# LPD-EPFL-ML/X-MAP

Measured on AMD Instinct MI355X. Metric: item_sim_pairs_per_s, higher is better.
Workload: dtype f64

## Files before the change

### include/xmap_hip.h

```cpp
#ifndef XMAP_HIP_H
#define XMAP_HIP_H
#include <stdint.h>

#ifdef __cplusplus
extern "C" {
#endif

#define XMAP_OK 0
#define XMAP_ERR_HIP -1
#define XMAP_ERR_ARG -2
#define XMAP_ERR_OVERFLOW -3
#define XMAP_ERR_CAPACITY -4

#define XMAP_COSINE 0
#define XMAP_ADJUST_COSINE 1
#define XMAP_COSINE_EXACT 2

#define XMAP_TOPC 10

typedef struct xmap_ratings {
    int64_t n_users;
    int32_t n_items;
    int64_t nnz;
    const int64_t *user_ptr;
// ... 156 lines not shown
    const int32_t *mutu;
    const int32_t *nij;
    const double *info;
    const double *frac;
} xmap_sim;

int xmap_bridge_flags(void *stream, const xmap_sim *S, const int32_t *prefix_cls, uint8_t *bb);

int xmap_knn_classify(void *stream, const xmap_sim *S, int top_k, const uint8_t *bb, const int32_t *suffix_cls,
                      const uint32_t *contains_mask, uint8_t *cls, int32_t *kcnt ,
                      int32_t *kcol , double *kval ,
                      int32_t row_lo, int32_t row_hi );

int xmap_knn_thresholds(void *stream, int32_t n_items, int top_k, const int32_t *kcnt, const int32_t *kcol, const double *kval,
                        void *thr );
int xmap_reverse_count(void *stream, const xmap_sim *S, int mode, int top_k, const uint8_t *bb, const uint8_t *cls,
                       const int32_t *kcnt, const int32_t *kcol, const double *kval, const int32_t *suffix_cls,
                       const uint32_t *contains_mask, const uint8_t *flags, const int64_t *attach_ptr,
                       const void *thr ,
                       int32_t *long_rows ,
                       uint8_t *eflag ,
                       int32_t *rcnt , int32_t row_lo, int32_t row_hi );
int xmap_reverse_count_att_rnn(void *stream, const xmap_sim *S, int top_k, const uint8_t *bb, const uint8_t *cls,
                               const int32_t *kcnt, const int32_t *kcol, const double *kval, const int32_t *suffix_cls,
                               const uint32_t *contains_mask, const uint8_t *flags, const void *thr, int32_t *long_rows,
                               uint8_t *eflag, int32_t *rcnt_att , int32_t *rcnt_rnn , int32_t row_lo, int32_t row_hi);
int xmap_reverse_fill(void *stream, const xmap_sim *S, int mode, int top_k, const uint8_t *bb, const uint8_t *cls,
                      const int32_t *kcnt, const int32_t *kcol, const double *kval, const int32_t *suffix_cls,
                      const uint32_t *contains_mask, const uint8_t *flags, const int64_t *attach_ptr,
                      const void *thr ,
                      int32_t *long_rows ,
                      uint8_t *eflag , const int64_t *rptr ,
                      int32_t *ridx, double *rval , uint8_t *rflag, int32_t row_lo, int32_t row_hi);

typedef struct xmap_ext_tables {
    int32_t n_items, top_k;
    const uint8_t *cls; const int32_t *kcnt; const int32_t *kcol; const double *kval; const uint8_t *flags;
    const int64_t *att_ptr; const int32_t *att_idx; const double *att_val;
    const int64_t *src_ptr; const int32_t *src_idx; const double *src_val; const uint8_t *src_flag;
    const int64_t *rnn_ptr; const int32_t *rnn_idx; const double *rnn_val;
    int32_t n_nb; const int32_t *nb_id; const int32_t *nb_list; const void *midX; const void *dir; const int64_t *dir_ptr;
    int32_t n_ends; const int32_t *urank; const int32_t *uitem;
} xmap_ext_tables;
typedef struct xmap_path_units {
    int32_t n_units; const int32_t *unit_start; const int32_t *unit_c; const int32_t *unit_G; const int32_t *unit_row;
    int32_t *unit_nt; int32_t n_heavy; const int32_t *heavy_unit0;
// ... 500 lines not shown
```

### x-map_amd/csrc/api.hip

```cpp
#include <math.h>
#include <stdlib.h>
#include <algorithm>
#include <vector>

#include "common.h"
#include "rec_model.h"

namespace xmap {

struct Pool {
    std::vector<void *> ptrs;
    void release() {
        for (void *p : ptrs) (void)hipFree(p);
        ptrs.clear();
    }
};
struct ScratchPool : Pool { ~ScratchPool() { release(); } };

}

using namespace xmap;

struct xmap_ctx {
    int device = 0;
// ... 135 lines not shown

static void drop_labels(xmap_ctx *c) {
    c->p_lab.release();
    c->have_lab = false;
    c->n_labels = 0; c->n_lab = 0;
    c->h_lab_ptr.clear();
}

static void drop_fold(xmap_ctx *c) {
    c->p_fold.release();
    c->have_fold = false;
    c->f_users = c->f_rows = 0;
}

static int reverse_list(xmap_ctx *c, int mode, const uint8_t *bb, const int64_t *attach_ptr, const void *thr, int32_t *long_rows,
                        uint8_t *eflag, int32_t *counted ,
                        const int64_t **rptr, const int32_t **ridx, const double **rval, const uint8_t **rflag) {
    const int I = c->R.n_items, k = c->top_k;
    int32_t *rcnt = counted;
    int64_t *ptr;
    XM_ALLOCZ(c->p_ext, ptr, I + 1);
    if (!counted) {
        XM_ALLOCZ(c->p_ext, rcnt, I);
        XM_TRY(xmap_reverse_count(c->st, &c->S, mode, k, bb, c->T.cls, c->T.kcnt, c->T.kcol, c->T.kval, c->R.suffix_cls,
                                  c->R.contains_mask, c->R.flags, attach_ptr, thr, long_rows, eflag, rcnt, 0, I));
    }
    int64_t n = 0;
    XM_TRY(xmap_exclusive_scan_i32_to_i64(c->st, rcnt, ptr, I, &n));
    int32_t *idx;
    double *val;
    uint8_t *flag;
    XM_ALLOC(c->p_ext, idx, n);
    XM_ALLOC(c->p_ext, val, 3 * (size_t)(n ? n : 1));
    XM_ALLOCZ(c->p_ext, flag, n);
    XM_TRY(xmap_reverse_fill(c->st, &c->S, mode, k, bb, c->T.cls, c->T.kcnt, c->T.kcol, c->T.kval, c->R.suffix_cls,
                             c->R.contains_mask, c->R.flags, attach_ptr, thr, long_rows, eflag, ptr, idx, val, flag, 0, I));
    *rptr = ptr; *ridx = idx; *rval = val; *rflag = flag;
    return XMAP_OK;
}

static int ensure_rows(xmap_ctx *c, int64_t slots, int64_t len, int64_t hrows) {
    if (c->acc == nullptr || c->acc_slots < slots || c->acc_len != len || c->hacc_rows < hrows) {
        c->p_rows.release();
        c->acc = nullptr; c->hacc = nullptr;
        XM_ALLOCZ(c->p_rows, c->acc, (size_t)slots * len * 4);
        XM_ALLOC(c->p_rows, c->touched, (size_t)slots * len);
        if (hrows) {
            XM_ALLOCZ(c->p_rows, c->hacc, (size_t)hrows * len * 4);
            XM_ALLOC(c->p_rows, c->htouched, (size_t)hrows * len);
        }
        c->acc_slots = slots; c->acc_len = len; c->hacc_rows = hrows;
// ... 340 lines not shown
    XM_ALLOCZ(c->p_ext, c->top_val, (size_t)I * XMAP_TOPC);
    c->n_out = c->n_paths = 0;
    if (I == 0) { c->have_ext = true; if (n_out) *n_out = 0; if (n_paths) *n_paths = 0; return XMAP_OK; }
    uint8_t *bb, *cls;
    int32_t *kcnt, *kcol;
    double *kval;
    XM_ALLOCZ(c->p_ext, bb, I); XM_ALLOC(c->p_ext, cls, I); XM_ALLOC(c->p_ext, kcnt, (size_t)I * 2);
    XM_ALLOC(c->p_ext, kcol, (size_t)I * 2 * k); XM_ALLOC(c->p_ext, kval, (size_t)I * 2 * k * 3);
    XM_TRY(xmap_bridge_flags(c->st, &c->S, c->R.prefix_cls, bb));
    XM_TRY(xmap_knn_classify(c->st, &c->S, k, bb, c->R.suffix_cls, c->R.contains_mask, cls, kcnt, kcol, kval, 0, I));
    T.cls = cls; T.kcnt = kcnt; T.kcol = kcol; T.kval = kval;
    XM_TRY(xmap_edge_ranges(c->st, &c->S, &c->fast_div));
    double *thr;
    int32_t *long_rows;
    XM_ALLOC(c->p_ext, thr, (size_t)I * 4);
    XM_ALLOC(c->p_ext, long_rows, I + 1);
    uint8_t *eflag;
    XM_ALLOC(c->p_ext, eflag, (size_t)(c->n_kept > 0 ? c->n_kept : 1));
    XM_TRY(xmap_knn_thresholds(c->st, I, k, kcnt, kcol, kval, thr));
    const uint8_t *dummy;
    int32_t *cnt_att, *cnt_rnn;
    XM_ALLOCZ(c->p_ext, cnt_att, I);
    XM_ALLOCZ(c->p_ext, cnt_rnn, I);
    XM_TRY(xmap_reverse_count_att_rnn(c->st, &c->S, k, bb, cls, kcnt, kcol, kval, c->R.suffix_cls, c->R.contains_mask, c->R.flags,
                                      thr, long_rows, eflag, cnt_att, cnt_rnn, 0, I));
    XM_TRY(reverse_list(c, 0, bb, nullptr, thr, long_rows, eflag, cnt_att, &T.att_ptr, &T.att_idx, &T.att_val, &dummy));
    XM_TRY(reverse_list(c, 2, bb, nullptr, thr, long_rows, eflag, cnt_rnn, &T.rnn_ptr, &T.rnn_idx, &T.rnn_val, &dummy));
    XM_TRY(reverse_list(c, 1, bb, T.att_ptr, thr, long_rows, eflag, nullptr, &T.src_ptr, &T.src_idx, &T.src_val, &T.src_flag));
    int64_t *wtmp, *P;
    XM_ALLOCZ(c->p_ext, wtmp, (size_t)4 * I); XM_ALLOCZ(c->p_ext, P, I);
    XM_TRY(xmap_path_weights(c->st, &T, wtmp, P));
    int32_t *nb_list, *nb_id;
    int64_t n_nb = 0;
    XM_ALLOC(c->p_ext, nb_list, I); XM_ALLOC(c->p_ext, nb_id, I);
    XM_TRY(xmap_nb_index(c->st, I, cls, nb_list, nb_id, &n_nb));
    T.n_nb = (int32_t)n_nb; T.nb_list = nb_list; T.nb_id = nb_id;
    if (n_nb > 0) {
        int32_t *ng;
        int64_t *nrec, *dir_ptr, *rec_ptr, n_tiles = 0, n_records = 0;
        void *dir, *midX;
        XM_ALLOC(c->p_ext, ng, n_nb); XM_ALLOC(c->p_ext, nrec, n_nb); XM_ALLOCZ(c->p_ext, dir_ptr, n_nb + 1); XM_ALLOCZ(c->p_ext, rec_ptr, n_nb + 1);
        XM_TRY(xmap_mid_rows_count(c->st, &T, ng, nrec));
        XM_TRY(xmap_exclusive_scan_i32_to_i64(c->st, ng, dir_ptr, n_nb, &n_tiles));
// ... 1655 lines not shown
```

### x-map_amd/csrc/reverse.hip

```cpp
#include "paths.h"
#include <stdlib.h>

namespace xmap {

struct RevArgs {
    int I, k, mode;
    int row_lo, row_hi;
    const KnnThr *thr;
    const int *long_rows;
    uint8_t *eflag;
    int rev_long;
    const long long *row_ptr;
    const int *col;
    const double *sim;
    const int *mutu;
    const int *nij;
    const double *info;
    const double *frac;
    const uint8_t *bb;
    const uint8_t *cls;
    const int *kcnt;
    const int *kcol;
    const double *kval;
    const int *suffix_cls;
// ... 73 lines not shown
        if (p < hi) A.eflag[p - p0] = (uint8_t)((ok ? (A.mode == 2 ? 4 : 1) : 0) | (fl << 1));
        return ok;
    }
    b = 0; sv = 0.0; fl = 0;
    bool ok = false;
    if (p < hi) {
        const uint8_t e = A.eflag[p - p0];
        ok = (e & (A.mode == 2 ? 4 : 1)) != 0;
        fl = (uint8_t)((e >> 1) & 1);
        if (ok) { b = A.col[p]; sv = A.sim[p]; }
    }
    return ok;
}

constexpr int REV_LONG = 4096;
constexpr int REV_WAVES = 16;
template <bool FILL>
__global__ __launch_bounds__(256) void k_reverse(RevArgs A) {
    int a = A.row_lo + blockIdx.x * 4 + (threadIdx.x >> 6);
    if (a >= A.row_hi) return;
    int lane = lane_id();
    long long lo = A.row_ptr[a], hi = A.row_ptr[a + 1];
    if (A.long_rows && hi - lo > A.rev_long) return;
    bool row_ok = true;
    if (A.mode == 1) row_ok = (A.flags[a] & 2) != 0;
    long long out = FILL ? A.rptr[a] : 0;
    int total = 0, total2 = 0;
    const long long p0 = A.eflag ? A.row_ptr[A.row_lo] : 0;
    if (row_ok)
        for (long long base = lo; base < hi; base += 64) {
            long long p = base + lane;
            int b; double sv; uint8_t fl;
            const bool ok = rev_test<FILL>(A, a, p, hi, p0, b, sv, fl);
            unsigned long long m = __ballot(ok);
            if (FILL && ok) rev_write(A, a, p, out + __popcll(m & lanemask_lt()), b, sv, fl);
            int c = __popcll(m);
            out += c;
            total += c;
            if (!FILL && A.mode == 3) total2 += __popcll(__ballot((fl & 2) != 0));
        }
    if (!FILL && lane == 0) { A.rcnt[a] = total; if (A.mode == 3) A.rcnt2[a] = total2; }
}

__global__ __launch_bounds__(256) void k_rev_long_rows(int row_lo, int row_hi, const long long *row_ptr, int rev_long,
                                                       int *long_rows ) {
    const int a = row_lo + blockIdx.x * blockDim.x + threadIdx.x;
    if (a < row_hi && row_ptr[a + 1] - row_ptr[a] > rev_long) long_rows[1 + atomicAdd(&long_rows[0], 1)] = a;
}

template <bool FILL>
__global__ __launch_bounds__(64 * REV_WAVES) void k_reverse_long(RevArgs A) {
    __shared__ int s_cnt[REV_WAVES];
    __shared__ int s_tot2;
    const int lane = lane_id(), w = threadIdx.x >> 6;
    const int n_long = A.long_rows[0];
    const long long p0 = A.eflag ? A.row_ptr[A.row_lo] : 0;
    for (int r = blockIdx.x; r < n_long; r += gridDim.x) {
        const int a = A.long_rows[1 + r];
        const long long lo = A.row_ptr[a], hi = A.row_ptr[a + 1];
        const bool row_ok = (A.mode != 1) || ((A.flags[a] & 2) != 0);
        long long out = FILL ? A.rptr[a] : 0;
        int total = 0, total2 = 0;
        if (!FILL && A.mode == 3) { if (threadIdx.x == 0) s_tot2 = 0; __syncthreads(); }
        if (row_ok)
            for (long long base = lo; base < hi; base += 64 * REV_WAVES) {
                const long long p = base + threadIdx.x;
                int b; double sv; uint8_t fl;
                const bool ok = rev_test<FILL>(A, a, p, hi, p0, b, sv, fl);
                const unsigned long long m = __ballot(ok);
                if (!FILL && A.mode == 3) total2 += __popcll(__ballot((fl & 2) != 0));
                if (lane == 0) s_cnt[w] = __popcll(m);
                __syncthreads();
                int before = 0, all = 0;
                for (int o = 0; o < REV_WAVES; o++) { const int c = s_cnt[o]; if (o < w) before += c; all += c; }
                if (FILL && ok) rev_write(A, a, p, out + before + __popcll(m & lanemask_lt()), b, sv, fl);
                out += all;
                total += all;
                __syncthreads();
            }
        if (!FILL && A.mode == 3) {
            if (lane == 0) atomicAdd(&s_tot2, total2);
            __syncthreads();
            if (threadIdx.x == 0) A.rcnt2[a] = s_tot2;
            __syncthreads();
        }
        if (!FILL && threadIdx.x == 0) A.rcnt[a] = total;
    }
}

}

using namespace xmap;

extern "C" {

static int reverse_common(void *stream, bool fill, const xmap_sim *S, int mode, int top_k, const uint8_t *bb,
                          const uint8_t *cls, const int32_t *kcnt, const int32_t *kcol, const double *kval,
                          const int32_t *suffix_cls, const uint32_t *contains_mask, const uint8_t *flags,
                          const int64_t *attach_ptr, const void *thr, int32_t *long_rows, uint8_t *eflag, int32_t *rcnt,
                          const int64_t *rptr, int32_t *ridx, double *rval, uint8_t *rflag, int32_t row_lo, int32_t row_hi,
                          int32_t *rcnt2 = nullptr) {
    XM_ARG(S && bb && cls && kcnt && kcol && kval && suffix_cls && contains_mask && flags);
    XM_ARG((mode >= 0 && mode <= 2) || (mode == 3 && !fill && rcnt2 && eflag));
    XM_ARG(mode != 1 || attach_ptr);
    XM_ARG(row_lo >= 0 && row_lo <= row_hi && row_hi <= S->n_items);
    if (row_hi == row_lo) return XMAP_OK;
    RevArgs A;
    A.I = S->n_items; A.k = top_k; A.mode = mode; A.thr = (const KnnThr *)thr; A.long_rows = long_rows; A.eflag = eflag;
    A.row_lo = row_lo; A.row_hi = row_hi;
    const char *rl = getenv("XMAP_REV_LONG");
    A.rev_long = (rl && atoi(rl) > 0) ? atoi(rl) : REV_LONG;
    A.row_ptr = (const long long *)S->row_ptr; A.col = S->col; A.sim = S->sim; A.mutu = S->mutu; A.nij = S->nij;
    A.info = S->info; A.frac = S->frac; A.bb = bb; A.cls = cls; A.kcnt = kcnt; A.kcol = kcol; A.kval = kval;
    A.suffix_cls = suffix_cls; A.contains_mask = contains_mask; A.flags = flags;
    A.attach_ptr = (const long long *)attach_ptr;
    A.rcnt2 = rcnt2;
    A.rcnt = rcnt; A.rptr = (const long long *)rptr; A.ridx = ridx; A.rval = rval; A.rflag = rflag;
    const int n_rows = row_hi - row_lo;
    dim3 grid((unsigned)((n_rows + 3) / 4)), block(256);
    hipStream_t st = (hipStream_t)stream;

    if (long_rows && !fill) {
        XM_HIP(hipMemsetAsync(long_rows, 0, sizeof(int32_t), st));
        k_rev_long_rows<<<dim3((unsigned)((n_rows + 255) / 256)), dim3(256), 0, st>>>(row_lo, row_hi, (const long long *)S->row_ptr,
                                                                                  A.rev_long, long_rows);
        XM_LAUNCH_CHECK();
    }
    if (fill) k_reverse<true><<<grid, block, 0, st>>>(A);
    else k_reverse<false><<<grid, block, 0, st>>>(A);
    XM_LAUNCH_CHECK();
    if (long_rows) {
        if (fill) k_reverse_long<true><<<dim3(512), dim3(64 * REV_WAVES), 0, st>>>(A);
        else k_reverse_long<false><<<dim3(512), dim3(64 * REV_WAVES), 0, st>>>(A);
        XM_LAUNCH_CHECK();
    }
    return XMAP_OK;
}

int xmap_reverse_count(void *stream, const xmap_sim *S, int mode, int top_k, const uint8_t *bb, const uint8_t *cls,
                       const int32_t *kcnt, const int32_t *kcol, const double *kval, const int32_t *suffix_cls,
                       const uint32_t *contains_mask, const uint8_t *flags, const int64_t *attach_ptr, const void *thr,
                       int32_t *long_rows, uint8_t *eflag, int32_t *rcnt, int32_t row_lo, int32_t row_hi) {
    XM_ARG(rcnt);
    return reverse_common(stream, false, S, mode, top_k, bb, cls, kcnt, kcol, kval, suffix_cls, contains_mask, flags,
                          attach_ptr, thr, long_rows, eflag, rcnt, nullptr, nullptr, nullptr, nullptr, row_lo, row_hi);
}

int xmap_reverse_count_att_rnn(void *stream, const xmap_sim *S, int top_k, const uint8_t *bb, const uint8_t *cls,
                               const int32_t *kcnt, const int32_t *kcol, const double *kval, const int32_t *suffix_cls,
                               const uint32_t *contains_mask, const uint8_t *flags, const void *thr, int32_t *long_rows,
                               uint8_t *eflag, int32_t *rcnt_att, int32_t *rcnt_rnn, int32_t row_lo, int32_t row_hi) {
    XM_ARG(rcnt_att && rcnt_rnn && eflag);
    return reverse_common(stream, false, S, 3, top_k, bb, cls, kcnt, kcol, kval, suffix_cls, contains_mask, flags, nullptr, thr,
                          long_rows, eflag, rcnt_att, nullptr, nullptr, nullptr, nullptr, row_lo, row_hi, rcnt_rnn);
}

int xmap_reverse_fill(void *stream, const xmap_sim *S, int mode, int top_k, const uint8_t *bb, const uint8_t *cls,
                      const int32_t *kcnt, const int32_t *kcol, const double *kval, const int32_t *suffix_cls,
                      const uint32_t *contains_mask, const uint8_t *flags, const int64_t *attach_ptr, const void *thr,
                      int32_t *long_rows, uint8_t *eflag, const int64_t *rptr, int32_t *ridx, double *rval, uint8_t *rflag,
                      int32_t row_lo, int32_t row_hi) {
    XM_ARG(rptr && ridx && rval);
    return reverse_common(stream, true, S, mode, top_k, bb, cls, kcnt, kcol, kval, suffix_cls, contains_mask, flags,
                          attach_ptr, thr, long_rows, eflag, nullptr, rptr, ridx, rval, rflag, row_lo, row_hi);
}

}
```

### x-map_amd/csrc/util.hip

```cpp
#include <stdarg.h>
#include <stdlib.h>
#include <vector>

#include "common.h"

namespace xmap {
static thread_local char g_err[512] = "";
void set_error(const char *fmt, ...) {
    va_list ap;
    va_start(ap, fmt);
    vsnprintf(g_err, sizeof(g_err), fmt, ap);
    va_end(ap);
}

namespace {
struct Chunk { char *base; size_t size, used; };
struct Arena { int dev; hipStream_t st; std::vector<Chunk> chunks; size_t live; };
thread_local std::vector<Arena> g_arenas;
constexpr size_t ARENA_KEEP = (size_t)256 << 20;
Arena *arena_find(int dev, hipStream_t st) {
    for (Arena &a : g_arenas) if (a.dev == dev && a.st == st) return &a;
    return nullptr;
}
Arena *arena_of(hipStream_t st) {
// ... 252 lines not shown
            XM_LAUNCH_CHECK();
        }
        XM_HIP(xm_free_async(tile, st));
    }
    if (h_total) {
        XM_HIP(hipMemcpyAsync(h_total, out0 + n, sizeof(int64_t), hipMemcpyDeviceToHost, st));
        if (n_arrays == 2) XM_HIP(hipMemcpyAsync(h_total + 1, out1 + n, sizeof(int64_t), hipMemcpyDeviceToHost, st));
        XM_HIP(hipStreamSynchronize(st));
    }
    return XMAP_OK;
}
}

extern "C" {
const char *xmap_last_error(void) { return xmap::g_err; }
int xmap_version(void) { return 125; }

int xmap_trim(void) {
    XM_HIP(hipDeviceSynchronize());
    int dev = 0;
    XM_HIP(hipGetDevice(&dev));
    for (xmap::Arena &a : xmap::g_arenas) {
        if (a.dev != dev || a.live != 0) continue;
        for (xmap::Chunk &c : a.chunks) (void)hipFree(c.base);
        a.chunks.clear();
    }
    return XMAP_OK;
}

int xmap_debug_arena(void *stream, int64_t *live, int64_t *reserved) {
    XM_ARG(live && reserved);
// ... 38 lines not shown
```

### x-map_amd/xmap/engine/device.py

```python
import ctypes as C
import math
import os

import numpy as np
import torch

from . import hipabi as abi
from .exactness import plain_sums_exact

lib = abi.lib
vp, i32, i64, check = abi.vp, abi.i32, abi.i64, abi.check


def _stream(dev):
    return C.c_void_p(torch.cuda.current_stream(dev).cuda_stream)


SLOT_TARGET = 768
CH_MIN = 2048
STEPWISE = os.environ.get("XMAP_STAGE_A_STEPWISE") == "1"


class DeviceRatings(object):

# ... 748 lines not shown
        E.cls = alloc(max(I, 1), torch.uint8)
        E.kcnt = alloc((max(I, 1), 2), torch.int32)
        E.kcol = alloc((max(I, 1), 2, k), torch.int32)
        E.kval = alloc((max(I, 1), 2, k, 3), torch.float64)
        with self.timed("knn_classify"):
            lo, hi = (0, I) if rows is None else (int(rows[0]), int(rows[1]))
            check(lib.xmap_knn_classify(st, C.byref(S.c), k, vp(E.bb), vp(R.suffix_cls), vp(R.contains_mask),
                                        vp(E.cls), vp(E.kcnt), vp(E.kcol), vp(E.kval), i32(lo), i32(hi)))
        return E

    def _reverse(self, S, E, mode, attach_ptr):
        st8 = self.reverse_count(S, E, mode, attach_ptr, None)
        self.reverse_fill(st8)
        return st8.out

    def reverse_count(self, S, E, mode, attach_ptr, rows):
        R = self.R
        I = R.n_items
        st8 = ExtResult()
        st8.S, st8.E, st8.mode = S, E, mode
        st8.rows = (0, I) if rows is None else (int(rows[0]), int(rows[1]))
        st8.rcnt = self._zeros(max(I, 1), torch.int32)
        st8.eflag = self._empty(max(int(S.col.numel()), 1), torch.uint8)
        st8.args = (C.byref(S.c), mode, E.k, vp(E.bb), vp(E.cls), vp(E.kcnt), vp(E.kcol), vp(E.kval),
                    vp(R.suffix_cls), vp(R.contains_mask), vp(R.flags), vp(attach_ptr), vp(getattr(E, "thr", None)),
                    vp(getattr(E, "long_rows", None)), vp(st8.eflag))
        st8.keep = attach_ptr
        check(lib.xmap_reverse_count(_stream(self.dev), *st8.args, vp(st8.rcnt), i32(st8.rows[0]), i32(st8.rows[1])))
        return st8

    def reverse_count_pair(self, S, E, rows):
        R = self.R
        I = R.n_items
        lo, hi = (0, I) if rows is None else (int(rows[0]), int(rows[1]))
        eflag = self._empty(max(int(S.col.numel()), 1), torch.uint8)
        sts = []
        for mode in (0, 2):
            st8 = ExtResult()
            st8.S, st8.E, st8.mode, st8.rows = S, E, mode, (lo, hi)
            st8.rcnt = self._zeros(max(I, 1), torch.int32)
            st8.eflag = eflag
            st8.args = (C.byref(S.c), mode, E.k, vp(E.bb), vp(E.cls), vp(E.kcnt), vp(E.kcol), vp(E.kval),
                        vp(R.suffix_cls), vp(R.contains_mask), vp(R.flags), vp(None), vp(E.thr),
                        vp(getattr(E, "long_rows", None)), vp(eflag))
            st8.keep = None
            sts.append(st8)
        check(lib.xmap_reverse_count_att_rnn(_stream(self.dev), C.byref(S.c), E.k, vp(E.bb), vp(E.cls), vp(E.kcnt), vp(E.kcol),
                                             vp(E.kval), vp(R.suffix_cls), vp(R.contains_mask), vp(R.flags), vp(E.thr),
                                             vp(getattr(E, "long_rows", None)), vp(eflag), vp(sts[0].rcnt), vp(sts[1].rcnt),
                                             i32(lo), i32(hi)))
        return sts

    def reverse_gather_counts(self, sts, comm):
        I = self.R.n_items
        lo, hi = sts[0].rows
        for st8, c in zip(sts, comm.all_gather_multi([st8.rcnt[lo:hi] for st8 in sts])):
            st8.rcnt[:I] = c

    def reverse_fill(self, st8):
        I = self.R.n_items
        st = _stream(self.dev)
        rptr = self._zeros(I + 1, torch.int64)
        tot = C.c_int64(0)
        check(lib.xmap_exclusive_scan_i32_to_i64(st, vp(st8.rcnt), vp(rptr), i64(I), C.byref(tot)))
# ... 242 lines not shown
        lo, hi = rows
        with self.timed("knn_gather"):
            k = E.k
            fd = torch.tensor([E.fast_div], dtype=torch.int64, device=self.dev)
            comm.all_reduce(fd, "min")
            E.fast_div = int(fd.item())
            cls, kcnt, kcol, kval = comm.all_gather_multi([E.cls[lo:hi], E.kcnt[lo:hi].reshape(-1), E.kcol[lo:hi].reshape(-1),
                                                           E.kval[lo:hi].reshape(-1)])
            E.cls[:I] = cls
            E.kcnt[:I] = kcnt.view(I, 2)
            E.kcol[:I] = kcol.view(I, 2, k)
            E.kval[:I] = kval.view(I, 2, k, 3)
        E.rows = None
        return E

    def ext_thresholds(self, E):
        I = self.R.n_items
        E.thr = self._empty(max(I, 1) * 4, torch.float64)
        check(lib.xmap_knn_thresholds(_stream(self.dev), i32(I), E.k, vp(E.kcnt), vp(E.kcol), vp(E.kval), vp(E.thr)))
        E.long_rows = self._empty(max(I, 1) + 1, torch.int32)

    def ext_reverse(self, S, E):
        with self.timed("reverse"):
            self.ext_thresholds(E)
            if getattr(E, "thr", None) is not None and os.environ.get("XMAP_REV_SEPARATE") != "1":
                st_att, st_rnn = self.reverse_count_pair(S, E, None)
                self.reverse_fill(st_att)
                self.reverse_fill(st_rnn)
                E.att, E.rnn = st_att.out, st_rnn.out
            else:
                E.att = self._reverse(S, E, 0, None)
                E.rnn = self._reverse(S, E, 2, None)
            E.src = self._reverse(S, E, 1, E.att[0])
        return E

    def ext_tables_from_knn(self, top_k, cls, kcnt, kcol, kval):
        R = self.R
        I, k = R.n_items, int(top_k)
        dev = self.dev
# ... 1174 lines not shown
```

### x-map_amd/xmap/engine/hipabi.py

```python
import ctypes as C
import os

HERE = os.path.dirname(os.path.abspath(__file__))
LIB_PATH = os.environ.get("XMAP_HIP_LIB") or os.path.normpath(os.path.join(HERE, "..", "..", "libxmap_hip.so"))
XLIB_PATH = os.environ.get("XMAP_HIP_XLIB") or os.path.normpath(os.path.join(HERE, "..", "..", "libxmap_hip_xcheck.so"))

COSINE, ADJUST_COSINE = 0, 1
METHODS = {"cosine": COSINE, "adjust_cosine": ADJUST_COSINE}
COSINE_EXACT = 2
TOPC = 10
MID_ROWS_SPAN = 36864
ERR_HIP, ERR_ARG, ERR_OVERFLOW, ERR_CAPACITY = -1, -2, -3, -4
TOPN_KEEP_HELD = 1
AUDIENCE_KEEP_HOLDERS = 1
SRC_RESIDENT, SRC_FOLDIN, SRC_ITEM_FOLDIN = 0, 1, 2
GROUP_MEAN, GROUP_MIN, GROUP_MAX = 0, 1, 2
GROUP_MAX_MEMBERS = 64
PEERS_SAME, PEERS_KEEP_SELF, PEERS_CENTRED = 1, 2, 4
UKNN_OWN_MEAN, UKNN_KEEP_HELD = 1, 2
RELATED_SUM, RELATED_MEAN, RELATED_MAX = 0, 1, 2
RELATED_KEEP_MEMBERS = 1
RELATED_HOW = {"sum": RELATED_SUM, "mean": RELATED_MEAN, "max": RELATED_MAX}
POP_COUNT, POP_MEAN = 0, 1
FILL_WINDOW = 4096
# ... 74 lines not shown

class RecFilter(C.Structure):
    _fields_ = [("allow", C.c_void_p), ("ex_ptr", C.c_void_p), ("ex_id", C.c_void_p), ("min_score", C.c_double)]


class FuseList(C.Structure):
    _fields_ = [("cnt", C.c_void_p), ("item", C.c_void_p), ("score", C.c_void_p), ("width", C.c_int32), ("weight", C.c_double)]


EXPORTS = [
    "xmap_last_error", "xmap_version", "xmap_trim", "xmap_debug_arena", "xmap_debug_arena_call", "xmap_debug_sort_pairs", "xmap_debug_record_chunks", "xmap_exclusive_scan_i64", "xmap_exclusive_scan_i32_to_i64",
    "xmap_exclusive_scan2_i32_to_i64", "xmap_scan_self_tiles", "xmap_sim3_plan_begin", "xmap_sim3_plan_wait", "xmap_sim3_counters_begin", "xmap_sim3_counters_wait",
    "xmap_build_csc", "xmap_user_stats", "xmap_item_stats", 
    "xmap_sim2_layout", "xmap_sim2_plan", "xmap_sim2_units",
    "xmap_sim2_pairs", "xmap_sim2_scatter", "xmap_sim3_layout", "xmap_sim3_plan", "xmap_sim3_mircount", "xmap_sim3_mirror", "xmap_item_partials", "xmap_item_merge", "xmap_sim2_pack_partials",
    "xmap_sim2_sort_partials", "xmap_sim2_merge_partials", "xmap_sim2_pack_pairs", "xmap_sim2_unpack_pairs", "xmap_bridge_flags", "xmap_knn_classify", "xmap_knn_thresholds", "xmap_reverse_count", "xmap_reverse_count_att_rnn",
    "xmap_reverse_fill", "xmap_topc_from_lists", "xmap_path_weights", "xmap_extend_paths", 
    "xmap_mid_rows_count", "xmap_mid_rows_place", "xmap_edge_ranges", "xmap_end_universe", "xmap_extend_cols", "xmap_extend_cols_slots", "xmap_nb_index", "xmap_path_plan", "xmap_end_order", "xmap_dense_normalize", "xmap_dense_layout", "xmap_dense_topk", "xmap_rec_select", "xmap_predict", "xmap_rec_profiles", "xmap_predict_rows", "xmap_mae", "xmap_topn_rows", "xmap_audience_rows", "xmap_explain_rows", "xmap_explain_sources", "xmap_eval_users", "xmap_topn_eval", "xmap_select_map", "xmap_alterego_count", "xmap_alterego_fill", "xmap_foldin_count", "xmap_foldin_fill", "xmap_union_count", "xmap_union_fill",
    "xmap_feed_text", "xmap_feed_texts", "xmap_feed_merge", "xmap_feed_sizes", "xmap_feed_arrays", "xmap_feed_ids", "xmap_feed_free",
    "xmap_ctx_upload_feed", "xmap_feed_format", "xmap_ctx_create", "xmap_ctx_destroy", "xmap_check_ratings", "xmap_ctx_upload_ratings", "xmap_ctx_item_sim", "xmap_ctx_sim_download", "xmap_ctx_extend",
    "xmap_ctx_ext_download", "xmap_ctx_ext_lists", "xmap_ctx_candidates", "xmap_ctx_generate", "xmap_ctx_gen_download",
    "xmap_ctx_rec_sim", "xmap_ctx_rec_profiles_download", "xmap_ctx_rec_download", "xmap_ctx_rec_select", "xmap_ctx_rec_set_neighbors",
    "xmap_ctx_rec_neighbors_download", "xmap_ctx_predict", "xmap_ctx_recommend", "xmap_ctx_evaluate_topn",
    "xmap_ctx_foldin", "xmap_ctx_foldin_download", "xmap_ctx_foldin_recommend", "xmap_ctx_foldin_predict", "xmap_ctx_union",
    "xmap_ctx_explain", "xmap_ctx_foldin_explain", "xmap_ctx_audience", "xmap_ctx_foldin_audience",
    "xmap_itemfold_count", "xmap_itemfold_fill", "xmap_itemfold_audience_rows", "xmap_ctx_item_foldin", "xmap_ctx_item_foldin_download",
    "xmap_ctx_item_foldin_audience", "xmap_ctx_item_foldin_predict", "xmap_ctx_item_foldin_recommend",
    "xmap_topn_rows_filtered", "xmap_audience_rows_filtered", "xmap_ctx_recommend_filtered", "xmap_ctx_audience_filtered",
    "xmap_div_index", "xmap_diversify_rows", "xmap_ctx_recommend_diverse",
    "xmap_group_topn_rows", "xmap_ctx_recommend_group",
    "xmap_peer_index", "xmap_peer_centre", "xmap_peer_rows", "xmap_ctx_peers", "xmap_peer_rows_ls", "xmap_ctx_peers_ls",
# ... 135 lines not shown
```

### x-map_amd/xmap/engine/sharded.py

```python
import os

import numpy as np
import torch


def balanced_ranges(weights, world):
    w = np.asarray(weights, dtype=np.float64)
    n = len(w)
    c = np.concatenate([[0.0], np.cumsum(w)])
    total = c[-1]
    cuts = [0]
    for r in range(1, world):
        target = total * r / world
        cuts.append(int(min(max(np.searchsorted(c, target, side="left"), cuts[-1]), n)))
    cuts.append(n)
    return [(cuts[r], cuts[r + 1]) for r in range(world)]


def unit_cuts(c, w_heavy, world):
    n = int(c.numel())
    if n == 0:
        return np.zeros(world + 1, np.int64)
    wh = w_heavy if w_heavy is not None else torch.zeros((), dtype=torch.float64, device=c.device)
    first = torch.minimum(((c[-1] + wh) / world - wh).clamp(min=0.0), c[-1])
# ... 314 lines not shown
            err = e
        comm.agree(err, "stage B (mirror)")
        if share is not None:
            comm.all_reduce(bb, "max")
        err = None
        try:
            E = eng.ext_knn(S, k, comm, rows=share, bb=bb)
        except Exception as e:
            err = e
        comm.agree(err, "stage B (knn tables)")
        eng.ext_gather(E, comm)
        rows = getattr(E, "row_share", None)
        with eng.timed("reverse"):
            err = None
            try:
                eng.ext_thresholds(E)
            except Exception as e:
                err = e
            comm.agree(err, "stage B (list thresholds)")
            for group in (((0, "att"), (2, "rnn")), ((1, "src"),)):
                err, sts = None, []
                try:
                    if len(group) == 2:
                        sts = eng.reverse_count_pair(S, E, rows)
                    else:
                        for mode, _ in group:
                            sts.append(eng.reverse_count(S, E, mode, E.att[0] if mode == 1 else None, rows))
                except Exception as e:
                    err = e
                comm.agree(err, "stage B (reverse lists: count)")
                if rows is not None:
# ... 25 lines not shown
```

Baseline: 28.86 billion.

## Split long reverse-list rows into fixed segments processed by independent waves

```diff
diff --git a/include/xmap_hip.h b/include/xmap_hip.h
--- a/include/xmap_hip.h
+++ b/include/xmap_hip.h
@@ -194,22 +194,23 @@
 
 int xmap_knn_thresholds(void *stream, int32_t n_items, int top_k, const int32_t *kcnt, const int32_t *kcol, const double *kval,
                         void *thr );
+int xmap_reverse_scratch_len(int32_t n_items, int64_t n_entries, int64_t *h_len);
 int xmap_reverse_count(void *stream, const xmap_sim *S, int mode, int top_k, const uint8_t *bb, const uint8_t *cls,
                        const int32_t *kcnt, const int32_t *kcol, const double *kval, const int32_t *suffix_cls,
                        const uint32_t *contains_mask, const uint8_t *flags, const int64_t *attach_ptr,
                        const void *thr ,
-                       int32_t *long_rows ,
+                       int32_t *long_rows , int64_t long_len ,
                        uint8_t *eflag ,
                        int32_t *rcnt , int32_t row_lo, int32_t row_hi );
 int xmap_reverse_count_att_rnn(void *stream, const xmap_sim *S, int top_k, const uint8_t *bb, const uint8_t *cls,
                                const int32_t *kcnt, const int32_t *kcol, const double *kval, const int32_t *suffix_cls,
                                const uint32_t *contains_mask, const uint8_t *flags, const void *thr, int32_t *long_rows,
-                               uint8_t *eflag, int32_t *rcnt_att , int32_t *rcnt_rnn , int32_t row_lo, int32_t row_hi);
+                               int64_t long_len, uint8_t *eflag, int32_t *rcnt_att , int32_t *rcnt_rnn , int32_t row_lo, int32_t row_hi);
 int xmap_reverse_fill(void *stream, const xmap_sim *S, int mode, int top_k, const uint8_t *bb, const uint8_t *cls,
                       const int32_t *kcnt, const int32_t *kcol, const double *kval, const int32_t *suffix_cls,
                       const uint32_t *contains_mask, const uint8_t *flags, const int64_t *attach_ptr,
                       const void *thr ,
-                      int32_t *long_rows ,
+                      int32_t *long_rows , int64_t long_len,
                       uint8_t *eflag , const int64_t *rptr ,
                       int32_t *ridx, double *rval , uint8_t *rflag, int32_t row_lo, int32_t row_hi);
 
diff --git a/x-map_amd/csrc/api.hip b/x-map_amd/csrc/api.hip
--- a/x-map_amd/csrc/api.hip
+++ b/x-map_amd/csrc/api.hip
@@ -173,7 +173,7 @@
 }
 
 static int reverse_list(xmap_ctx *c, int mode, const uint8_t *bb, const int64_t *attach_ptr, const void *thr, int32_t *long_rows,
-                        uint8_t *eflag, int32_t *counted ,
+                        int64_t long_len, uint8_t *eflag, int32_t *counted ,
                         const int64_t **rptr, const int32_t **ridx, const double **rval, const uint8_t **rflag) {
     const int I = c->R.n_items, k = c->top_k;
     int32_t *rcnt = counted;
@@ -182,7 +182,7 @@
     if (!counted) {
         XM_ALLOCZ(c->p_ext, rcnt, I);
         XM_TRY(xmap_reverse_count(c->st, &c->S, mode, k, bb, c->T.cls, c->T.kcnt, c->T.kcol, c->T.kval, c->R.suffix_cls,
-                                  c->R.contains_mask, c->R.flags, attach_ptr, thr, long_rows, eflag, rcnt, 0, I));
+                                  c->R.contains_mask, c->R.flags, attach_ptr, thr, long_rows, long_len, eflag, rcnt, 0, I));
     }
     int64_t n = 0;
     XM_TRY(xmap_exclusive_scan_i32_to_i64(c->st, rcnt, ptr, I, &n));
@@ -193,7 +193,8 @@
     XM_ALLOC(c->p_ext, val, 3 * (size_t)(n ? n : 1));
     XM_ALLOCZ(c->p_ext, flag, n);
     XM_TRY(xmap_reverse_fill(c->st, &c->S, mode, k, bb, c->T.cls, c->T.kcnt, c->T.kcol, c->T.kval, c->R.suffix_cls,
-                             c->R.contains_mask, c->R.flags, attach_ptr, thr, long_rows, eflag, ptr, idx, val, flag, 0, I));
+                             c->R.contains_mask, c->R.flags, attach_ptr, thr, long_rows, long_len, eflag, ptr, idx, val, flag, 0,
+                             I));
     *rptr = ptr; *ridx = idx; *rval = val; *rflag = flag;
     return XMAP_OK;
 }
@@ -564,7 +565,9 @@
     double *thr;
     int32_t *long_rows;
     XM_ALLOC(c->p_ext, thr, (size_t)I * 4);
-    XM_ALLOC(c->p_ext, long_rows, I + 1);
+    int64_t long_len = 0;
+    XM_TRY(xmap_reverse_scratch_len(I, c->n_kept > 0 ? c->n_kept : 0, &long_len));
+    XM_ALLOC(c->p_ext, long_rows, (size_t)long_len);
     uint8_t *eflag;
     XM_ALLOC(c->p_ext, eflag, (size_t)(c->n_kept > 0 ? c->n_kept : 1));
     XM_TRY(xmap_knn_thresholds(c->st, I, k, kcnt, kcol, kval, thr));
@@ -573,10 +576,10 @@
     XM_ALLOCZ(c->p_ext, cnt_att, I);
     XM_ALLOCZ(c->p_ext, cnt_rnn, I);
     XM_TRY(xmap_reverse_count_att_rnn(c->st, &c->S, k, bb, cls, kcnt, kcol, kval, c->R.suffix_cls, c->R.contains_mask, c->R.flags,
-                                      thr, long_rows, eflag, cnt_att, cnt_rnn, 0, I));
-    XM_TRY(reverse_list(c, 0, bb, nullptr, thr, long_rows, eflag, cnt_att, &T.att_ptr, &T.att_idx, &T.att_val, &dummy));
-    XM_TRY(reverse_list(c, 2, bb, nullptr, thr, long_rows, eflag, cnt_rnn, &T.rnn_ptr, &T.rnn_idx, &T.rnn_val, &dummy));
-    XM_TRY(reverse_list(c, 1, bb, T.att_ptr, thr, long_rows, eflag, nullptr, &T.src_ptr, &T.src_idx, &T.src_val, &T.src_flag));
+                                      thr, long_rows, long_len, eflag, cnt_att, cnt_rnn, 0, I));
+    XM_TRY(reverse_list(c, 0, bb, nullptr, thr, long_rows, long_len, eflag, cnt_att, &T.att_ptr, &T.att_idx, &T.att_val, &dummy));
+    XM_TRY(reverse_list(c, 2, bb, nullptr, thr, long_rows, long_len, eflag, cnt_rnn, &T.rnn_ptr, &T.rnn_idx, &T.rnn_val, &dummy));
+    XM_TRY(reverse_list(c, 1, bb, T.att_ptr, thr, long_rows, long_len, eflag, nullptr, &T.src_ptr, &T.src_idx, &T.src_val, &T.src_flag));
     int64_t *wtmp, *P;
     XM_ALLOCZ(c->p_ext, wtmp, (size_t)4 * I); XM_ALLOCZ(c->p_ext, P, I);
     XM_TRY(xmap_path_weights(c->st, &T, wtmp, P));
diff --git a/x-map_amd/csrc/reverse.hip b/x-map_amd/csrc/reverse.hip
--- a/x-map_amd/csrc/reverse.hip
+++ b/x-map_amd/csrc/reverse.hip
@@ -8,6 +8,11 @@
     int row_lo, row_hi;
     const KnnThr *thr;
     const int *long_rows;
+    int seg_len, seg_cap;
+    int *seg_first;
+    const int2 *seg_item;
+    int *seg_cnt;
+    int *seg_cnt2;
     uint8_t *eflag;
     int rev_long;
     const long long *row_ptr;
@@ -111,7 +116,25 @@
 }
 
 constexpr int REV_LONG = 4096;
-constexpr int REV_WAVES = 16;
+constexpr int REV_SEG = 1024;
+
+template <bool FILL>
+__device__ __forceinline__ void rev_walk(const RevArgs &A, int a, long long lo, long long hi, long long p0, long long out,
+                                         int &total, int &total2) {
+    const int lane = lane_id();
+    for (long long base = lo; base < hi; base += 64) {
+        long long p = base + lane;
+        int b; double sv; uint8_t fl;
+        const bool ok = rev_test<FILL>(A, a, p, hi, p0, b, sv, fl);
+        unsigned long long m = __ballot(ok);
+        if (FILL && ok) rev_write(A, a, p, out + __popcll(m & lanemask_lt()), b, sv, fl);
+        int c = __popcll(m);
+        out += c;
+        total += c;
+        if (!FILL && A.mode == 3) total2 += __popcll(__ballot((fl & 2) != 0));
+    }
+}
+
 template <bool FILL>
 __global__ __launch_bounds__(256) void k_reverse(RevArgs A) {
     int a = A.row_lo + blockIdx.x * 4 + (threadIdx.x >> 6);
@@ -121,67 +144,71 @@
     if (A.long_rows && hi - lo > A.rev_long) return;
     bool row_ok = true;
     if (A.mode == 1) row_ok = (A.flags[a] & 2) != 0;
-    long long out = FILL ? A.rptr[a] : 0;
     int total = 0, total2 = 0;
     const long long p0 = A.eflag ? A.row_ptr[A.row_lo] : 0;
-    if (row_ok)
-        for (long long base = lo; base < hi; base += 64) {
-            long long p = base + lane;
-            int b; double sv; uint8_t fl;
-            const bool ok = rev_test<FILL>(A, a, p, hi, p0, b, sv, fl);
-            unsigned long long m = __ballot(ok);
-            if (FILL && ok) rev_write(A, a, p, out + __popcll(m & lanemask_lt()), b, sv, fl);
-            int c = __popcll(m);
-            out += c;
-            total += c;
-            if (!FILL && A.mode == 3) total2 += __popcll(__ballot((fl & 2) != 0));
+    if (row_ok) rev_walk<FILL>(A, a, lo, hi, p0, FILL ? A.rptr[a] : 0, total, total2);
+    if (!FILL && lane == 0) { A.rcnt[a] = total; if (A.mode == 3) A.rcnt2[a] = total2; }
+}
+
+struct RevSeg {
+    static long long head(int I) { return 2 + 2 * (long long)I; }
+    static long long cap(int I, long long len) { return len > head(I) ? (len - head(I)) / 5 : 0; }
+    static long long len(int I, long long n_entries, int seg_len) { return head(I) + 5 * (n_entries / seg_len + I + 1); }
+};
+
+__global__ __launch_bounds__(256) void k_rev_long_rows(int row_lo, int row_hi, const long long *row_ptr, int rev_long, int seg_len,
+                                                       int seg_cap, int *long_rows , int *seg_first,
+                                                       int2 *seg_item) {
+    const int a = row_lo + blockIdx.x * blockDim.x + threadIdx.x;
+    if (a >= row_hi) return;
+    const long long n = row_ptr[a + 1] - row_ptr[a];
+    if (n <= rev_long) return;
+    const int r = atomicAdd(&long_rows[0], 1);
+    long_rows[2 + r] = a;
+    const int ns = (int)((n + seg_len - 1) / seg_len);
+    const int s0 = atomicAdd(&long_rows[1], ns);
+    seg_first[r] = s0;
+    for (int j = 0; j < ns && s0 + j < seg_cap; j++) seg_item[s0 + j] = make_int2(a, j);
+}
+
+template <bool FILL>
+__global__ __launch_bounds__(256) void k_reverse_seg(RevArgs A) {
+    const int lane = lane_id();
+    const int n_seg = A.long_rows[1] < A.seg_cap ? A.long_rows[1] : A.seg_cap;
+    const long long p0 = A.eflag ? A.row_ptr[A.row_lo] : 0;
+    for (int s = blockIdx.x * 4 + (threadIdx.x >> 6); s < n_seg; s += gridDim.x * 4) {
+        const int2 it = A.seg_item[s];
+        const int a = it.x;
+        const long long lo = A.row_ptr[a] + (long long)it.y * A.seg_len;
+        long long hi = A.row_ptr[a + 1];
+        if (hi - lo > A.seg_len) hi = lo + A.seg_len;
+        const bool row_ok = (A.mode != 1) || ((A.flags[a] & 2) != 0);
+        int total = 0, total2 = 0;
+        if (row_ok) rev_walk<FILL>(A, a, lo, hi, p0, FILL ? A.rptr[a] + A.seg_cnt[s] : 0, total, total2);
+        if (!FILL && lane == 0) { A.seg_cnt[s] = total; if (A.mode == 3) A.seg_cnt2[s] = total2; }
+    }
+}
+
+__global__ __launch_bounds__(256) void k_rev_seg_scan(RevArgs A) {
+    const int lane = lane_id();
+    const int n_long = A.long_rows[0];
+    for (int r = blockIdx.x * 4 + (threadIdx.x >> 6); r < n_long; r += gridDim.x * 4) {
+        const int a = A.long_rows[2 + r];
+        const int ns = (int)((A.row_ptr[a + 1] - A.row_ptr[a] + A.seg_len - 1) / A.seg_len), s0 = A.seg_first[r];
+        for (int l = 0; l < (A.mode == 3 ? 2 : 1); l++) {
+            int *cnt = l ? A.seg_cnt2 : A.seg_cnt;
+            int run = 0;
+            for (int j0 = 0; j0 < ns; j0 += 64) {
+                const int s = s0 + j0 + lane;
+                const bool in = j0 + lane < ns && s < A.seg_cap;
+                const int v = in ? cnt[s] : 0;
+                int incl = v;
+                for (int d = 1; d < 64; d <<= 1) { const int o = __shfl_up(incl, d, 64); if (lane >= d) incl += o; }
+                if (in) cnt[s] = run + incl - v;
+                run += rl32(incl, 63);
+            }
+            if (lane == 0) (l ? A.rcnt2 : A.rcnt)[a] = run;
         }
-    if (!FILL && lane == 0) { A.rcnt[a] = total; if (A.mode == 3) A.rcnt2[a] = total2; }
-}
-
-__global__ __launch_bounds__(256) void k_rev_long_rows(int row_lo, int row_hi, const long long *row_ptr, int rev_long,
-                                                       int *long_rows ) {
-    const int a = row_lo + blockIdx.x * blockDim.x + threadIdx.x;
-    if (a < row_hi && row_ptr[a + 1] - row_ptr[a] > rev_long) long_rows[1 + atomicAdd(&long_rows[0], 1)] = a;
-}
-
-template <bool FILL>
-__global__ __launch_bounds__(64 * REV_WAVES) void k_reverse_long(RevArgs A) {
-    __shared__ int s_cnt[REV_WAVES];
-    __shared__ int s_tot2;
-    const int lane = lane_id(), w = threadIdx.x >> 6;
-    const int n_long = A.long_rows[0];
-    const long long p0 = A.eflag ? A.row_ptr[A.row_lo] : 0;
-    for (int r = blockIdx.x; r < n_long; r += gridDim.x) {
-        const int a = A.long_rows[1 + r];
-        const long long lo = A.row_ptr[a], hi = A.row_ptr[a + 1];
-        const bool row_ok = (A.mode != 1) || ((A.flags[a] & 2) != 0);
-        long long out = FILL ? A.rptr[a] : 0;
-        int total = 0, total2 = 0;
-        if (!FILL && A.mode == 3) { if (threadIdx.x == 0) s_tot2 = 0; __syncthreads(); }
-        if (row_ok)
-            for (long long base = lo; base < hi; base += 64 * REV_WAVES) {
-                const long long p = base + threadIdx.x;
-                int b; double sv; uint8_t fl;
-                const bool ok = rev_test<FILL>(A, a, p, hi, p0, b, sv, fl);
-                const unsigned long long m = __ballot(ok);
-                if (!FILL && A.mode == 3) total2 += __popcll(__ballot((fl & 2) != 0));
-                if (lane == 0) s_cnt[w] = __popcll(m);
-                __syncthreads();
-                int before = 0, all = 0;
-                for (int o = 0; o < REV_WAVES; o++) { const int c = s_cnt[o]; if (o < w) before += c; all += c; }
-                if (FILL && ok) rev_write(A, a, p, out + before + __popcll(m & lanemask_lt()), b, sv, fl);
-                out += all;
-                total += all;
-                __syncthreads();
-            }
-        if (!FILL && A.mode == 3) {
-            if (lane == 0) atomicAdd(&s_tot2, total2);
-            __syncthreads();
-            if (threadIdx.x == 0) A.rcnt2[a] = s_tot2;
-            __syncthreads();
-        }
-        if (!FILL && threadIdx.x == 0) A.rcnt[a] = total;
     }
 }
 
@@ -189,18 +216,32 @@
 
 using namespace xmap;
 
+static int rev_seg_len() {
+    const char *e = getenv("XMAP_REV_SEG");
+    const int v = (e && atoi(e) > 0) ? atoi(e) : REV_SEG;
+    return (v + 63) / 64 * 64;
+}
+
 extern "C" {
+
+int xmap_reverse_scratch_len(int32_t n_items, int64_t n_entries, int64_t *h_len) {
+    XM_ARG(n_items >= 0 && n_entries >= 0 && h_len);
+    *h_len = RevSeg::len(n_items, n_entries, rev_seg_len());
+    return XMAP_OK;
+}
 
 static int reverse_common(void *stream, bool fill, const xmap_sim *S, int mode, int top_k, const uint8_t *bb,
                           const uint8_t *cls, const int32_t *kcnt, const int32_t *kcol, const double *kval,
                           const int32_t *suffix_cls, const uint32_t *contains_mask, const uint8_t *flags,
-                          const int64_t *attach_ptr, const void *thr, int32_t *long_rows, uint8_t *eflag, int32_t *rcnt,
-                          const int64_t *rptr, int32_t *ridx, double *rval, uint8_t *rflag, int32_t row_lo, int32_t row_hi,
+                          const int64_t *attach_ptr, const void *thr, int32_t *long_rows, int64_t long_len, uint8_t *eflag,
+                          int32_t *rcnt, const int64_t *rptr, int32_t *ridx, double *rval, uint8_t *rflag, int32_t row_lo, int32_t row_hi,
                           int32_t *rcnt2 = nullptr) {
     XM_ARG(S && bb && cls && kcnt && kcol && kval && suffix_cls && contains_mask && flags);
     XM_ARG((mode >= 0 && mode <= 2) || (mode == 3 && !fill && rcnt2 && eflag));
     XM_ARG(mode != 1 || attach_ptr);
     XM_ARG(row_lo >= 0 && row_lo <= row_hi && row_hi <= S->n_items);
+    const long long seg_cap = long_rows ? RevSeg::cap(S->n_items, long_len) : 0;
+    XM_ARG(!long_rows || (seg_cap >= 1 && seg_cap <= 0x7fffffff && ((uintptr_t)long_rows & 7) == 0));
     if (row_hi == row_lo) return XMAP_OK;
     RevArgs A;
     A.I = S->n_items; A.k = top_k; A.mode = mode; A.thr = (const KnnThr *)thr; A.long_rows = long_rows; A.eflag = eflag;
@@ -213,23 +254,39 @@
     A.attach_ptr = (const long long *)attach_ptr;
     A.rcnt2 = rcnt2;
     A.rcnt = rcnt; A.rptr = (const long long *)rptr; A.ridx = ridx; A.rval = rval; A.rflag = rflag;
+    A.seg_len = rev_seg_len(); A.seg_cap = (int)seg_cap;
+    A.seg_first = nullptr; A.seg_item = nullptr; A.seg_cnt = A.seg_cnt2 = nullptr;
+    if (long_rows) {
+        int32_t *seg = long_rows + RevSeg::head(A.I);
+        A.seg_first = long_rows + 2 + A.I;
+        A.seg_item = (const int2 *)seg;
+        const int list = (mode == 1) ? 2 : (mode == 2) ? 1 : 0;
+        A.seg_cnt = seg + (2 + list) * seg_cap;
+        A.seg_cnt2 = seg + 3 * seg_cap;
+    }
     const int n_rows = row_hi - row_lo;
     dim3 grid((unsigned)((n_rows + 3) / 4)), block(256);
     hipStream_t st = (hipStream_t)stream;
 
     if (long_rows && !fill) {
-        XM_HIP(hipMemsetAsync(long_rows, 0, sizeof(int32_t), st));
-        k_rev_long_rows<<<dim3((unsigned)((n_rows + 255) / 256)), dim3(256), 0, st>>>(row_lo, row_hi, (const long long *)S->row_ptr,
-                                                                                  A.rev_long, long_rows);
+        XM_HIP(hipMemsetAsync(long_rows, 0, 2 * sizeof(int32_t), st));
+        k_rev_long_rows<<<dim3((unsigned)((n_rows + 255) / 256)), dim3(256), 0, st>>>(
+            row_lo, row_hi, (const long long *)S->row_ptr, A.rev_long, A.seg_len, A.seg_cap, long_rows, A.seg_first,
+            (int2 *)(long_rows + RevSeg::head(A.I)));
         XM_LAUNCH_CHECK();
     }
     if (fill) k_reverse<true><<<grid, block, 0, st>>>(A);
     else k_reverse<false><<<grid, block, 0, st>>>(A);
     XM_LAUNCH_CHECK();
     if (long_rows) {
-        if (fill) k_reverse_long<true><<<dim3(512), dim3(64 * REV_WAVES), 0, st>>>(A);
-        else k_reverse_long<false><<<dim3(512), dim3(64 * REV_WAVES), 0, st>>>(A);
+        const dim3 sgrid((unsigned)((seg_cap + 3) / 4 < 4096 ? (seg_cap + 3) / 4 : 4096));
+        if (fill) k_reverse_seg<true><<<sgrid, block, 0, st>>>(A);
+        else k_reverse_seg<false><<<sgrid, block, 0, st>>>(A);
         XM_LAUNCH_CHECK();
+        if (!fill) {
+            k_rev_seg_scan<<<dim3((unsigned)((n_rows + 3) / 4 < 256 ? (n_rows + 3) / 4 : 256)), block, 0, st>>>(A);
+            XM_LAUNCH_CHECK();
+        }
     }
     return XMAP_OK;
 }
@@ -237,29 +294,29 @@
 int xmap_reverse_count(void *stream, const xmap_sim *S, int mode, int top_k, const uint8_t *bb, const uint8_t *cls,
                        const int32_t *kcnt, const int32_t *kcol, const double *kval, const int32_t *suffix_cls,
                        const uint32_t *contains_mask, const uint8_t *flags, const int64_t *attach_ptr, const void *thr,
-                       int32_t *long_rows, uint8_t *eflag, int32_t *rcnt, int32_t row_lo, int32_t row_hi) {
+                       int32_t *long_rows, int64_t long_len, uint8_t *eflag, int32_t *rcnt, int32_t row_lo, int32_t row_hi) {
     XM_ARG(rcnt);
     return reverse_common(stream, false, S, mode, top_k, bb, cls, kcnt, kcol, kval, suffix_cls, contains_mask, flags,
-                          attach_ptr, thr, long_rows, eflag, rcnt, nullptr, nullptr, nullptr, nullptr, row_lo, row_hi);
+                          attach_ptr, thr, long_rows, long_len, eflag, rcnt, nullptr, nullptr, nullptr, nullptr, row_lo, row_hi);
 }
 
 int xmap_reverse_count_att_rnn(void *stream, const xmap_sim *S, int top_k, const uint8_t *bb, const uint8_t *cls,
                                const int32_t *kcnt, const int32_t *kcol, const double *kval, const int32_t *suffix_cls,
                                const uint32_t *contains_mask, const uint8_t *flags, const void *thr, int32_t *long_rows,
-                               uint8_t *eflag, int32_t *rcnt_att, int32_t *rcnt_rnn, int32_t row_lo, int32_t row_hi) {
+                               int64_t long_len, uint8_t *eflag, int32_t *rcnt_att, int32_t *rcnt_rnn, int32_t row_lo, int32_t row_hi) {
     XM_ARG(rcnt_att && rcnt_rnn && eflag);
     return reverse_common(stream, false, S, 3, top_k, bb, cls, kcnt, kcol, kval, suffix_cls, contains_mask, flags, nullptr, thr,
-                          long_rows, eflag, rcnt_att, nullptr, nullptr, nullptr, nullptr, row_lo, row_hi, rcnt_rnn);
+                          long_rows, long_len, eflag, rcnt_att, nullptr, nullptr, nullptr, nullptr, row_lo, row_hi, rcnt_rnn);
 }
 
 int xmap_reverse_fill(void *stream, const xmap_sim *S, int mode, int top_k, const uint8_t *bb, const uint8_t *cls,
                       const int32_t *kcnt, const int32_t *kcol, const double *kval, const int32_t *suffix_cls,
                       const uint32_t *contains_mask, const uint8_t *flags, const int64_t *attach_ptr, const void *thr,
-                      int32_t *long_rows, uint8_t *eflag, const int64_t *rptr, int32_t *ridx, double *rval, uint8_t *rflag,
-                      int32_t row_lo, int32_t row_hi) {
+                      int32_t *long_rows, int64_t long_len, uint8_t *eflag, const int64_t *rptr, int32_t *ridx, double *rval,
+                      uint8_t *rflag, int32_t row_lo, int32_t row_hi) {
     XM_ARG(rptr && ridx && rval);
     return reverse_common(stream, true, S, mode, top_k, bb, cls, kcnt, kcol, kval, suffix_cls, contains_mask, flags,
-                          attach_ptr, thr, long_rows, eflag, nullptr, rptr, ridx, rval, rflag, row_lo, row_hi);
-}
-
-}
+                          attach_ptr, thr, long_rows, long_len, eflag, nullptr, rptr, ridx, rval, rflag, row_lo, row_hi);
+}
+
+}
diff --git a/x-map_amd/csrc/util.hip b/x-map_amd/csrc/util.hip
--- a/x-map_amd/csrc/util.hip
+++ b/x-map_amd/csrc/util.hip
@@ -290,7 +290,7 @@
 
 extern "C" {
 const char *xmap_last_error(void) { return xmap::g_err; }
-int xmap_version(void) { return 125; }
+int xmap_version(void) { return 126; }
 
 int xmap_trim(void) {
     XM_HIP(hipDeviceSynchronize());
diff --git a/x-map_amd/xmap/engine/device.py b/x-map_amd/xmap/engine/device.py
--- a/x-map_amd/xmap/engine/device.py
+++ b/x-map_amd/xmap/engine/device.py
@@ -786,6 +786,11 @@
         self.reverse_fill(st8)
         return st8.out
 
+    @staticmethod
+    def _long_rows(E):
+        t = getattr(E, "long_rows", None)
+        return vp(t), i64(0 if t is None else t.numel())
+
     def reverse_count(self, S, E, mode, attach_ptr, rows):
         R = self.R
         I = R.n_items
@@ -796,7 +801,7 @@
         st8.eflag = self._empty(max(int(S.col.numel()), 1), torch.uint8)
         st8.args = (C.byref(S.c), mode, E.k, vp(E.bb), vp(E.cls), vp(E.kcnt), vp(E.kcol), vp(E.kval),
                     vp(R.suffix_cls), vp(R.contains_mask), vp(R.flags), vp(attach_ptr), vp(getattr(E, "thr", None)),
-                    vp(getattr(E, "long_rows", None)), vp(st8.eflag))
+                    *self._long_rows(E), vp(st8.eflag))
         st8.keep = attach_ptr
         check(lib.xmap_reverse_count(_stream(self.dev), *st8.args, vp(st8.rcnt), i32(st8.rows[0]), i32(st8.rows[1])))
         return st8
@@ -814,12 +819,12 @@
             st8.eflag = eflag
             st8.args = (C.byref(S.c), mode, E.k, vp(E.bb), vp(E.cls), vp(E.kcnt), vp(E.kcol), vp(E.kval),
                         vp(R.suffix_cls), vp(R.contains_mask), vp(R.flags), vp(None), vp(E.thr),
-                        vp(getattr(E, "long_rows", None)), vp(eflag))
+                        *self._long_rows(E), vp(eflag))
             st8.keep = None
             sts.append(st8)
         check(lib.xmap_reverse_count_att_rnn(_stream(self.dev), C.byref(S.c), E.k, vp(E.bb), vp(E.cls), vp(E.kcnt), vp(E.kcol),
                                              vp(E.kval), vp(R.suffix_cls), vp(R.contains_mask), vp(R.flags), vp(E.thr),
-                                             vp(getattr(E, "long_rows", None)), vp(eflag), vp(sts[0].rcnt), vp(sts[1].rcnt),
+                                             *self._long_rows(E), vp(eflag), vp(sts[0].rcnt), vp(sts[1].rcnt),
                                              i32(lo), i32(hi)))
         return sts
 
@@ -1092,15 +1097,19 @@
         E.rows = None
         return E
 
-    def ext_thresholds(self, E):
+    def ext_thresholds(self, E, S=None):
         I = self.R.n_items
         E.thr = self._empty(max(I, 1) * 4, torch.float64)
         check(lib.xmap_knn_thresholds(_stream(self.dev), i32(I), E.k, vp(E.kcnt), vp(E.kcol), vp(E.kval), vp(E.thr)))
-        E.long_rows = self._empty(max(I, 1) + 1, torch.int32)
+        E.long_rows = None
+        if S is not None:
+            n = C.c_int64(0)
+            check(lib.xmap_reverse_scratch_len(i32(I), i64(S.col.numel()), C.byref(n)))
+            E.long_rows = self._empty(int(n.value), torch.int32)
 
     def ext_reverse(self, S, E):
         with self.timed("reverse"):
-            self.ext_thresholds(E)
+            self.ext_thresholds(E, S)
             if getattr(E, "thr", None) is not None and os.environ.get("XMAP_REV_SEPARATE") != "1":
                 st_att, st_rnn = self.reverse_count_pair(S, E, None)
                 self.reverse_fill(st_att)
diff --git a/x-map_amd/xmap/engine/hipabi.py b/x-map_amd/xmap/engine/hipabi.py
--- a/x-map_amd/xmap/engine/hipabi.py
+++ b/x-map_amd/xmap/engine/hipabi.py
@@ -112,7 +112,7 @@
     "xmap_build_csc", "xmap_user_stats", "xmap_item_stats", 
     "xmap_sim2_layout", "xmap_sim2_plan", "xmap_sim2_units",
     "xmap_sim2_pairs", "xmap_sim2_scatter", "xmap_sim3_layout", "xmap_sim3_plan", "xmap_sim3_mircount", "xmap_sim3_mirror", "xmap_item_partials", "xmap_item_merge", "xmap_sim2_pack_partials",
-    "xmap_sim2_sort_partials", "xmap_sim2_merge_partials", "xmap_sim2_pack_pairs", "xmap_sim2_unpack_pairs", "xmap_bridge_flags", "xmap_knn_classify", "xmap_knn_thresholds", "xmap_reverse_count", "xmap_reverse_count_att_rnn",
+    "xmap_sim2_sort_partials", "xmap_sim2_merge_partials", "xmap_sim2_pack_pairs", "xmap_sim2_unpack_pairs", "xmap_bridge_flags", "xmap_knn_classify", "xmap_knn_thresholds", "xmap_reverse_scratch_len", "xmap_reverse_count", "xmap_reverse_count_att_rnn",
     "xmap_reverse_fill", "xmap_topc_from_lists", "xmap_path_weights", "xmap_extend_paths", 
     "xmap_mid_rows_count", "xmap_mid_rows_place", "xmap_edge_ranges", "xmap_end_universe", "xmap_extend_cols", "xmap_extend_cols_slots", "xmap_nb_index", "xmap_path_plan", "xmap_end_order", "xmap_dense_normalize", "xmap_dense_layout", "xmap_dense_topk", "xmap_rec_select", "xmap_predict", "xmap_rec_profiles", "xmap_predict_rows", "xmap_mae", "xmap_topn_rows", "xmap_audience_rows", "xmap_explain_rows", "xmap_explain_sources", "xmap_eval_users", "xmap_topn_eval", "xmap_select_map", "xmap_alterego_count", "xmap_alterego_fill", "xmap_foldin_count", "xmap_foldin_fill", "xmap_union_count", "xmap_union_fill",
     "xmap_feed_text", "xmap_feed_texts", "xmap_feed_merge", "xmap_feed_sizes", "xmap_feed_arrays", "xmap_feed_ids", "xmap_feed_free",
diff --git a/x-map_amd/xmap/engine/sharded.py b/x-map_amd/xmap/engine/sharded.py
--- a/x-map_amd/xmap/engine/sharded.py
+++ b/x-map_amd/xmap/engine/sharded.py
@@ -352,7 +352,7 @@
         with eng.timed("reverse"):
             err = None
             try:
-                eng.ext_thresholds(E)
+                eng.ext_thresholds(E, S)
             except Exception as e:
                 err = e
             comm.agree(err, "stage B (list thresholds)")
```

New measurement: 28.72 billion. Within noise of the previous version (-0.5%).
